# cvxgrp/scs

Measured on AMD Instinct MI355X. Metric: ADMM iters/sec (+ time-to-eps=1e-4), 1e6-var random SOCP, 1 GPU, higher is better.
Workload: dtype f64

## Files before the change

### scs_amd/csrc/linsys.h

```cpp
#pragma once
#include "spmv.h"
#include "scs_host.h"
#include "spmv_wave.h"
#include "spmm.h"

namespace scsamd {

int selected_device();

struct CgCtl {
  real ztr[2];
  real norm_r;
  real tol;
  real rhs_norm;
  int zero_rhs;
  int cg_done;
  int iters;
  int max_its;
  unsigned seq;
};

typedef unsigned long long cg_word;
__host__ __device__ inline cg_word cg_word_pack(unsigned seq, int iters, int done) {
  return ((cg_word)seq << 32) | ((cg_word)(unsigned)iters << 1) | (cg_word)(done ? 1 : 0);
}

struct CgCtlM {
  real ztr[2][MULTI_W_MAX];
  real norm_r[MULTI_W_MAX], tol[MULTI_W_MAX], rhs_norm[MULTI_W_MAX];
  int zero_rhs[MULTI_W_MAX];
  int done[MULTI_W_MAX];
  int iters[MULTI_W_MAX];
  int max_its;
  int all_done;
};

struct MultiWork {
  int width = 0;
  int last_its = 16;
  DevBuf<real> bx, by;
  DevBuf<real> s, r, z, p;
  DevBuf<real> gt;
  DevBuf<real> Pp;
  DevBuf<real> part_pgp, part_ztr, part_max;
  DevBuf<CgCtlM> ctl;
  PinnedBuf<CgCtlM> hctl;
};

struct ShardHook {
  void *ctx = nullptr;
// ... 106 lines not shown
```

### scs_amd/csrc/linsys.hip

```cpp
#include "linsys.h"
#include <thread>
#include <exception>
#include <system_error>
#include <algorithm>
#include "spmv_wave_build.h"
#include "host_transpose.h"
#include <algorithm>
#include <atomic>
#include <chrono>

namespace scsamd {

constexpr int CG_GRAPH_ITERS = 8;
constexpr long long CG_GRAPH_MAX_NNZ = 2000000;
constexpr int CG_LEAD_DEFAULT = 4;
constexpr int CG_PACE_SPIN = 64;


constexpr int VEC_MAX_GRID = 512;
constexpr int PART_CAP = 4096;
static_assert(PART_CAP >= SPMV_MAX_GRID && PART_CAP >= WR_MAX_GRID && PART_CAP >= 2 * 512, "partial arrays too small");

CsrDev::~CsrDev() { delete wave; }

// ... 23 lines not shown

__global__ __launch_bounds__(SCSAMD_BLOCK) void k_rhs_prep(real *b, const real *__restrict__ ry,
                                                           real *tmp, int n, int m,
                                                           const real *part, int pcount, CgCtl *ctl,
                                                           real tol, const real *warm_part,
                                                           int warm_cnt, real warm_scale, int max_its, unsigned seq,
                                                           cg_word *prog) {
  __shared__ real red[4];
  const real nb = reduce_partials_max(part, pcount, red);
  const int gtid = blockIdx.x * blockDim.x + threadIdx.x, gs = gridDim.x * blockDim.x;
  const bool zero = nb <= (real)1e-12;
  if (zero) {
    for (int i = gtid; i < n + m; i += gs) b[i] = 0;
  } else {
    for (int i = gtid; i < m; i += gs) tmp[i] = b[n + i] / ry[i];
  }
  real t = tol;
  if (warm_part) {
    const real nw = reduce_partials_max(warm_part, warm_cnt, red) * warm_scale;
    t = t < nw ? t : nw;
    t = (real)0.2 * t;
    t = t > (real)1e-12 ? t : (real)1e-12;
  }
  if (gtid == 0) {
    ctl->zero_rhs = zero ? 1 : 0;
    ctl->cg_done = zero ? 1 : 0;
    ctl->iters = 0;
    ctl->max_its = max_its;
    ctl->tol = t;
    ctl->rhs_norm = nb;
    ctl->norm_r = 0;
    ctl->ztr[0] = 0;
    ctl->ztr[1] = 0;
    ctl->seq = seq;
    publish_progress(prog, seq, 0, zero ? 1 : 0);
  }
}

__global__ __launch_bounds__(SCSAMD_BLOCK) void k_cg_init(real *x, const real *__restrict__ s, real *r,
                                                          real *z, const real *__restrict__ M, int n,
                                                          real *part_ztr, real *part_max,
                                                          const CgCtl *ctl) {
  __shared__ real red[4];
  if (ctl->zero_rhs) return;
  real ztr = 0, mx = 0;
  for (int i = blockIdx.x * blockDim.x + threadIdx.x; i < n; i += gridDim.x * blockDim.x) {
    real ri;
    if (s) {
      ri = x[i] - r[i];
      x[i] = s[i];
    } else {
      ri = x[i];
      x[i] = 0;
    }
    r[i] = ri;
    const real zi = ri * M[i];
    z[i] = zi;
    ztr += zi * ri;
    const real a = absval(ri);
    mx = a > mx ? a : mx;
  }
  ztr = block_sum(ztr, red);
  mx = block_max(mx, red);
  if (threadIdx.x == 0) {
    part_ztr[blockIdx.x] = ztr;
    part_max[blockIdx.x] = mx;
  }
}

__global__ __launch_bounds__(SCSAMD_BLOCK) void k_cg_start(real *p, const real *__restrict__ z, int n,
                                                           const real *part_ztr, const real *part_max,
                                                           int pcount, CgCtl *ctl, cg_word *prog) {
  __shared__ real red[4];
  if (ctl->zero_rhs) return;
  const real ztr = reduce_partials_sum(part_ztr, pcount, red);
  const real nr = reduce_partials_max(part_max, pcount, red);
  const real tol = ctl->tol;
  const real thr = tol > (real)1e-12 ? tol : (real)1e-12;
  const bool conv = nr < thr;
  if (!conv)
    for (int i = blockIdx.x * blockDim.x + threadIdx.x; i < n; i += gridDim.x * blockDim.x) p[i] = z[i];
  if (blockIdx.x == 0 && threadIdx.x == 0) {
    ctl->ztr[0] = ztr;
    ctl->norm_r = nr;
    if (conv) {
      ctl->cg_done = 1;
      publish_progress(prog, ctl->seq, 0, 1);
    }
  }
}

__global__ __launch_bounds__(SCSAMD_BLOCK) void k_cg_update(real *x, real *r, real *z,
                                                            const real *__restrict__ p,
                                                            const real *__restrict__ Gp,
                                                            const real *__restrict__ M, int n,
                                                            const real *part_pgp, int cnt_pgp,
                                                            real *part_ztr, real *part_max,
                                                            const CgCtl *ctl, int parity, int ntm) {
  __shared__ real red[4];
  const int gtid = blockIdx.x * blockDim.x + threadIdx.x, gs = gridDim.x * blockDim.x;
  const int nv = n / RVW;
  const bool has = gtid < nv;
  rvec P0 = {}, G0 = {}, M0 = {}, X0 = {}, R0 = {};
  if (has) {
    P0 = ldv(p, gtid);
    G0 = ldv(Gp, gtid);
    M0 = ldv(M, gtid);
    X0 = ldv(x, gtid);
    R0 = ldv(r, gtid);
  }
  const int done = ctl->cg_done;
  const real ztr_in = ctl->ztr[parity];
  real psum = 0;
  for (int i = threadIdx.x; i < cnt_pgp; i += blockDim.x) psum += part_pgp[i];
  if (done) return;
  const real pgp = block_sum(psum, red);
  const real alpha = ztr_in / pgp;
  real ztr = 0, mx = 0;
  if (has) {
    rvec Z;
#pragma unroll
    for (int e = 0; e < RVW; ++e) {
      X0.v[e] += alpha * P0.v[e];
      const real ri = R0.v[e] + (-alpha) * G0.v[e];
      R0.v[e] = ri;
      const real zi = ri * M0.v[e];
      Z.v[e] = zi;
      ztr += zi * ri;
      const real a = absval(ri);
      mx = a > mx ? a : mx;
    }
    stv(x, gtid, X0);
    stv(r, gtid, R0);
    stv(z, gtid, Z);
  }
  int iv0 = gtid + gs;
  if (ntm & 4) {
    for (; iv0 + gs < nv; iv0 += 2 * gs) {
      const int ia = iv0, ib = iv0 + gs;
      const rvec Pa = ldv_nt(p, ia), Pb = ldv_nt(p, ib), Ga = ldv_nt(Gp, ia), Gb = ldv_nt(Gp, ib), Ma = ldv_nt(M, ia), Mb = ldv_nt(M, ib);
      rvec Xa = ldv_nt(x, ia), Xb = ldv_nt(x, ib), Ra = ldv_nt(r, ia), Rb = ldv_nt(r, ib), Za, Zb;
#pragma unroll
      for (int e = 0; e < RVW; ++e) {
        Xa.v[e] += alpha * Pa.v[e];
        const real ri = Ra.v[e] + (-alpha) * Ga.v[e];
        Ra.v[e] = ri;
        const real zi = ri * Ma.v[e];
        Za.v[e] = zi;
        ztr += zi * ri;
        const real a = absval(ri);
        mx = a > mx ? a : mx;
      }
#pragma unroll
      for (int e = 0; e < RVW; ++e) {
        Xb.v[e] += alpha * Pb.v[e];
        const real ri = Rb.v[e] + (-alpha) * Gb.v[e];
        Rb.v[e] = ri;
        const real zi = ri * Mb.v[e];
        Zb.v[e] = zi;
        ztr += zi * ri;
        const real a = absval(ri);
        mx = a > mx ? a : mx;
      }
      stv_nt(x, ia, Xa);
      stv_nt(r, ia, Ra);
      stv(z, ia, Za);
      stv_nt(x, ib, Xb);
      stv_nt(r, ib, Rb);
      stv(z, ib, Zb);
    }
  }
  for (int iv = iv0; iv < nv; iv += gs) {
    const rvec P = (ntm & 2) ? ldv_nt(p, iv) : ldv(p, iv), G = (ntm & 2) ? ldv_nt(Gp, iv) : ldv(Gp, iv), Mv = ntm ? ldv_nt(M, iv) : ldv(M, iv);
    rvec X = ntm ? ldv_nt(x, iv) : ldv(x, iv), R = ntm ? ldv_nt(r, iv) : ldv(r, iv), Z;
#pragma unroll
    for (int e = 0; e < RVW; ++e) {
      X.v[e] += alpha * P.v[e];
      const real ri = R.v[e] + (-alpha) * G.v[e];
      R.v[e] = ri;
      const real zi = ri * Mv.v[e];
      Z.v[e] = zi;
      ztr += zi * ri;
      const real a = absval(ri);
      mx = a > mx ? a : mx;
    }
    if (ntm) {
      stv_nt(x, iv, X);
      stv_nt(r, iv, R);
    } else {
      stv(x, iv, X);
      stv(r, iv, R);
    }
    if (ntm & 2) stv_nt(z, iv, Z);
    else stv(z, iv, Z);
  }
  for (int i = nv * RVW + gtid; i < n; i += gs) {
    const real pi = p[i], gi = Gp[i];
    x[i] += alpha * pi;
    const real ri = r[i] + (-alpha) * gi;
    r[i] = ri;
    const real zi = ri * M[i];
    z[i] = zi;
    ztr += zi * ri;
    const real a = absval(ri);
    mx = a > mx ? a : mx;
  }
  ztr = block_sum(ztr, red);
  mx = block_max(mx, red);
  if (threadIdx.x == 0) {
    part_ztr[blockIdx.x] = ztr;
    part_max[blockIdx.x] = mx;
  }
}

__global__ __launch_bounds__(SCSAMD_BLOCK) void k_cg_direction(real *p, const real *__restrict__ z, int n,
                                                               const real *part_ztr,
                                                               const real *part_max, int pcount,
                                                               CgCtl *ctl, int parity, int dmode, cg_word *prog) {
  __shared__ real red[4];
  const int gtid = blockIdx.x * blockDim.x + threadIdx.x, gs = gridDim.x * blockDim.x;
  const int nv = n / RVW;
  const bool has = gtid < nv;
  rvec Z0 = {}, P0 = {};
  if (has) {
    Z0 = ldv(z, gtid);
    P0 = ldv(p, gtid);
  }
  const int done = ctl->cg_done;
  const real ztr_prev = ctl->ztr[parity], tol = ctl->tol;
  real zs = 0, ms = 0;
  for (int i = threadIdx.x; i < pcount; i += blockDim.x) {
    zs += part_ztr[i];
    const real v = part_max[i];
    ms = v > ms ? v : ms;
  }
  if (done) return;
  const real ztr = block_sum(zs, red);
  const real nr = block_max(ms, red);
  const bool conv = nr < tol;
  const bool brk = !conv && ztr_prev == (real)0;
  if (!conv && !brk) {
    const real beta = ztr / ztr_prev;
    if (has) {
#pragma unroll
      for (int e = 0; e < RVW; ++e) P0.v[e] = Z0.v[e] + beta * P0.v[e];
      stv(p, gtid, P0);
    }
    int iv0 = gtid + gs;
    if (dmode & 4) {
      for (; iv0 + gs < nv; iv0 += 2 * gs) {
        const rvec Za = (dmode & 1) ? ldv_nt(z, iv0) : ldv(z, iv0), Zb = (dmode & 1) ? ldv_nt(z, iv0 + gs) : ldv(z, iv0 + gs);
        rvec Pa = ldv(p, iv0), Pb = ldv(p, iv0 + gs);
#pragma unroll
        for (int e = 0; e < RVW; ++e) {
          Pa.v[e] = Za.v[e] + beta * Pa.v[e];
          Pb.v[e] = Zb.v[e] + beta * Pb.v[e];
        }
        stv(p, iv0, Pa);
        stv(p, iv0 + gs, Pb);
      }
    }
    for (int iv = iv0; iv < nv; iv += gs) {
      const rvec Z = (dmode & 1) ? ldv_nt(z, iv) : ldv(z, iv);
      rvec P = ldv(p, iv);
#pragma unroll
      for (int e = 0; e < RVW; ++e) P.v[e] = Z.v[e] + beta * P.v[e];
      if (dmode & 2) stv_nt(p, iv, P);
      else stv(p, iv, P);
    }
    for (int i = nv * RVW + gtid; i < n; i += gs) p[i] = z[i] + beta * p[i];
  }
  if (blockIdx.x == 0 && threadIdx.x == 0) {
    ctl->ztr[parity ^ 1] = ztr;
    ctl->norm_r = nr;
    const int its = ctl->iters + (brk ? 0 : 1);
    const bool stop = conv || brk || its >= ctl->max_its;
    ctl->iters = its;
    if (stop) ctl->cg_done = 1;
    publish_progress(prog, ctl->seq, its, stop ? 1 : 0);
  }
}

__global__ __launch_bounds__(SCSAMD_BLOCK) void k_cg3_update(real *x, real *r, real *p, const real *__restrict__ Gp,
                                                             const real *__restrict__ M, int n, const real *part_pgp,
                                                             const real *part_d1, const real *part_d2, int cnt_sp,
                                                             const real *part_ztr_prev, const real *part_max_prev, int cnt_v,
                                                             real *part_ztr, real *part_max, CgCtl *ctl, int it, cg_word *prog) {
  __shared__ real red[4];
  const int gtid = blockIdx.x * blockDim.x + threadIdx.x, gs = gridDim.x * blockDim.x;
  const int nv = n / RVW;
  const bool has = gtid < nv;
  rvec P0 = {}, G0 = {}, M0 = {}, X0 = {}, R0 = {};
  if (has) {
    P0 = ldv(p, gtid);
    G0 = ldv(Gp, gtid);
    M0 = ldv_nt(M, gtid);
    X0 = ldv_nt(x, gtid);
    R0 = ldv_nt(r, gtid);
  }
  const int done = ctl->cg_done, max_its = ctl->max_its;
  const real tol = ctl->tol;
  real ztr = ctl->ztr[0];
  real s0 = 0, s1 = 0, s2 = 0, zs = 0, ms = 0;
// ... 402 lines not shown
      iters = (int)(it + 1);
    }
  }
  __syncthreads();
  for (int i = tid; i < m; i += FUSED_THREADS) b[n + i] = (-b[n + i] + fused_row(A, b, i)) / ry[i];
  if (tid == 0) {
    ctl->zero_rhs = 0; ctl->cg_done = 1; ctl->iters = iters; ctl->tol = t; ctl->rhs_norm = nb; ctl->norm_r = nr;
    ctl->ztr[0] = ztr; ctl->ztr[1] = 0;
    ctl->seq = seq;
  }
  __syncthreads();
  if (tid == 0) publish_progress(prog, seq, iters, 1);
}

LinSys::~LinSys() {
  if (cg_graph) (void)hipGraphExecDestroy(cg_graph);
  delete multi;
  if (own_stream && stream) (void)hipStreamDestroy(stream);
}

template <int E, int WPB, int MODE>
static void launch_lockstep_one(const WaveRowsDev &wd, int g, size_t lds, hipStream_t stream, const WaveView &v, const real *x, real *y,
                                const EpiArgs &e, const int *skip) {
  static std::atomic<unsigned long long> attr_set[4] = {};
  int dev = 0;
  HIP_CHECK(hipGetDevice(&dev));
  const bool tracked = dev >= 0 && dev < 256;
  const unsigned long long bit = 1ull << (dev & 63);
  if (!tracked || !(attr_set[(dev >> 6) & 3].load(std::memory_order_acquire) & bit)) {
    HIP_CHECK(hipFuncSetAttribute(reinterpret_cast<const void *>(csr_wave_lockstep_kernel<E, WPB, MODE>), hipFuncAttributeMaxDynamicSharedMemorySize,
                                  144 * 1024));
    if (tracked) attr_set[(dev >> 6) & 3].fetch_or(bit, std::memory_order_release);
  }
  hipLaunchKernelGGL((csr_wave_lockstep_kernel<E, WPB, MODE>), dim3(g), dim3(WPB * 64), lds, stream, v, x, y, e, skip, wd.accrows);
}
template <int E>
static void launch_lockstep(const WaveRowsDev &wd, int g, size_t lds, hipStream_t stream, const WaveView &v, const real *x, real *y,
                            const EpiArgs &e, const int *skip) {
#define LS_CASE(W, M)                                                                                                  \
  if (wd.ls_wpb == W && wd.ls_bmode == M) return launch_lockstep_one<E, W, M>(wd, g, lds, stream, v, x, y, e, skip);
  LS_CASE(16, 4) LS_CASE(16, 1) LS_CASE(8, 4) LS_CASE(8, 1)
#undef LS_CASE
  throw HipError("scs_amd: lockstep SpMV variant not instantiated");
}

void LinSys::launch_spmv(int epi, const CsrDev &mat, const real *x, real *y, const EpiArgs &e,
                         const int *skip) {
  int slot = -1;
  const bool sample = profiling && ((spmv_sample_ctr++ % 7) == 0);
  if (sample) slot = spmv_timer.start(stream);
  if (mat.wave && mat.wave->built) {
    const WaveRowsDev &wd = *mat.wave;
    const int g = wd.grid();
    const size_t lds = wd.lds_bytes();
    WaveView v = wd.view();
#define WR_LAUNCH(E)                                                                                                   \
  do {                                                                                                                 \
    if (wd.wide) {                                                                                                     \
      hipLaunchKernelGGL((csr_wave_wide_kernel<E>), dim3(g), dim3(WR_BLOCK), lds, stream, v, x, y, e, skip, wd.accrows);  \
    } else if (wd.lockstep) {                                                                                          \
      launch_lockstep<E>(wd, g, lds, stream, v, x, y, e, skip);                                                        \
    } else if (wd.pipelined == 1) hipLaunchKernelGGL((csr_wave_kernel<E, 1>), dim3(g), dim3(WR_BLOCK), lds, stream, v, x, y, e, skip, wd.accrows); \
    else if (wd.pipelined == 2) hipLaunchKernelGGL((csr_wave_kernel<E, 2>), dim3(g), dim3(WR_BLOCK), lds, stream, v, x, y, e, skip, wd.accrows); \
    else hipLaunchKernelGGL((csr_wave_kernel<E, 0>), dim3(g), dim3(WR_BLOCK), lds, stream, v, x, y, e, skip, wd.accrows);                       \
  } while (0)
    switch (epi) {
    case EPI_PLAIN: WR_LAUNCH(EPI_PLAIN); break;
    case EPI_DIV: WR_LAUNCH(EPI_DIV); break;
    case EPI_GP: WR_LAUNCH(EPI_GP); break;
    case EPI_ACC: WR_LAUNCH(EPI_ACC); break;
    case EPI_NEGDIV: WR_LAUNCH(EPI_NEGDIV); break;
    case EPI_GP3: WR_LAUNCH(EPI_GP3); break;
    default: throw HipError("scs_amd: bad spmv epilogue");
    }
#undef WR_LAUNCH
    if (sample) spmv_timer.stop(slot, stream);
    n_spmv++;
    return;
  }
  const int g = mat.grid();
  CsrView v = mat.view();
  switch (epi) {
  case EPI_PLAIN: hipLaunchKernelGGL(csr_stream_kernel<EPI_PLAIN>, dim3(g), dim3(SCSAMD_BLOCK), 0, stream, v, x, y, e, skip); break;
  case EPI_DIV: hipLaunchKernelGGL(csr_stream_kernel<EPI_DIV>, dim3(g), dim3(SCSAMD_BLOCK), 0, stream, v, x, y, e, skip); break;
  case EPI_GP: hipLaunchKernelGGL(csr_stream_kernel<EPI_GP>, dim3(g), dim3(SCSAMD_BLOCK), 0, stream, v, x, y, e, skip); break;
  case EPI_ACC: hipLaunchKernelGGL(csr_stream_kernel<EPI_ACC>, dim3(g), dim3(SCSAMD_BLOCK), 0, stream, v, x, y, e, skip); break;
  case EPI_NEGDIV: hipLaunchKernelGGL(csr_stream_kernel<EPI_NEGDIV>, dim3(g), dim3(SCSAMD_BLOCK), 0, stream, v, x, y, e, skip); break;
  default: throw HipError("scs_amd: bad spmv epilogue");
  }
  if (sample) spmv_timer.stop(slot, stream);
  n_spmv++;
}

static void host_transpose(int rows_out, int cols_out, const eoff *Ap, const int *Ai, const real *Ax, std::vector<eoff> &Cp, std::vector<int> &Ci,
                           std::vector<real> &Cx, bool force_serial = false) {
  host_transpose_t<eoff, real>(rows_out, cols_out, Ap, Ai, Ax, Cp, Ci, Cx, force_serial);
}
// ... 376 lines not shown
  real *p_cur = pbuf[it & 1];
  if (it == 0) {
    EpiArgs e1{ry.p, nullptr, nullptr, nullptr};
    launch_spmv(EPI_DIV, A, p_cur, tmp.p, e1, &c->cg_done);
  } else {
    const int q = (int)((it - 1) & 1);
    hipLaunchKernelGGL(k_cg2_a, dim3(A.grid()), dim3(SCSAMD_BLOCK), (size_t)n * sizeof(real), stream, A.view(), ry.p, tmp.p, cg_x,
                       rbuf[(it - 1) & 1], rbuf[it & 1], Gp.p, M.p, pbuf[(it - 1) & 1], p_cur, n, partA.p, gAt, gv, c, q, prog_dev);
    n_spmv++;
  }
  EpiArgs e2{rx.p, p_cur, nullptr, partA.p};
  launch_spmv(EPI_GP, At, tmp.p, Gp.p, e2, &c->cg_done);
}

void LinSys::enqueue_cg_iteration(int q) {
  CgCtl *c = ctl.p;
  const int gv = vec_grid(n);
  const int gAt = (At.wave && At.wave->built) ? At.wave->grid() : At.grid();
  real *part_pgp = partA.p, *part_ztr = partB.p, *part_max = partB.p + PART_CAP / 2;
  EpiArgs e1{ry.p, nullptr, nullptr, nullptr};
  launch_spmv(EPI_DIV, A, p.p, tmp.p, e1, &c->cg_done);
  if (has_P) {
    EpiArgs ep{nullptr, nullptr, nullptr, nullptr};
    launch_spmv(EPI_PLAIN, P, p.p, Pp.p, ep, &c->cg_done);
  }
  EpiArgs e2{rx.p, p.p, has_P ? Pp.p : nullptr, shard ? (real *)nullptr : part_pgp};
  launch_spmv(EPI_GP, At, tmp.p, Gp.p, e2, &c->cg_done);
  int cnt_pgp = gAt;
  if (shard) {
    shard_allreduce(Gp.p, (size_t)n, 0);
    hipLaunchKernelGGL(k_dot_partial, dim3(gv), dim3(SCSAMD_BLOCK), 0, stream, (const real *)p.p, (const real *)Gp.p, n, part_pgp, &c->cg_done);
    cnt_pgp = gv;
  }
  hipLaunchKernelGGL(k_cg_update, dim3(gv), dim3(SCSAMD_BLOCK), 0, stream, cg_x, r.p, z.p, p.p, Gp.p, M.p, n,
                     part_pgp, cnt_pgp, part_ztr, part_max, c, q, nt_mode);
  hipLaunchKernelGGL(k_cg_direction, dim3(gv), dim3(SCSAMD_BLOCK), 0, stream, p.p, z.p, n, part_ztr, part_max,
                     gv, c, q, dir_mode, prog_dev);
}

void LinSys::enqueue_cg3_iteration(long long it) {
  CgCtl *c = ctl.p;
  const int gv = vec_grid(n);
  const int gAt = At.wave->grid();
  const int q = (int)(it & 1);
  real *ztr_cur = partB.p + q * (PART_CAP / 4), *max_cur = partB.p + PART_CAP / 2 + q * (PART_CAP / 4);
  real *ztr_prev = partB.p + (q ^ 1) * (PART_CAP / 4), *max_prev = partB.p + PART_CAP / 2 + (q ^ 1) * (PART_CAP / 4);
  EpiArgs e1{ry.p, nullptr, nullptr, nullptr};
  launch_spmv(EPI_DIV, A, p.p, tmp.p, e1, &c->cg_done);
  if (has_P) {
    EpiArgs ep{nullptr, nullptr, nullptr, nullptr};
    launch_spmv(EPI_PLAIN, P, p.p, Pp.p, ep, &c->cg_done);
  }
  EpiArgs e2{rx.p, p.p, has_P ? Pp.p : nullptr, partA.p};
  e2.mv = M.p;
  e2.rv = r.p;
  e2.partial2 = partC.p;
  e2.partial3 = partD.p;
  launch_spmv(EPI_GP3, At, tmp.p, Gp.p, e2, &c->cg_done);
  hipLaunchKernelGGL(k_cg3_update, dim3(gv), dim3(SCSAMD_BLOCK), 0, stream, cg_x, r.p, p.p, Gp.p, M.p, n, partA.p, partC.p, partD.p, gAt,
                     ztr_prev, max_prev, gv, ztr_cur, max_cur, c, (int)std::min<long long>(it, 2147483647LL), prog_dev);
}

bool LinSys::build_cg_graph() {
  cg_graph_tried = true;
  hipGraph_t g = nullptr;
  if (hipStreamBeginCapture(stream, hipStreamCaptureModeRelaxed) != hipSuccess) {
    (void)hipGetLastError();
    return false;
  }
  bool ok = true;
// ... 530 lines not shown
```

### scs_amd/csrc/spmv_wave.h

```cpp
#pragma once
#include "spmv.h"
#include <algorithm>

namespace scsamd {

constexpr int WR_WPB = 4;
constexpr int WR_BLOCK = WR_WPB * 64;
constexpr int WR_ROWS_MAX = 1024;
constexpr int WR_MAX_GRID = 4096;
constexpr int WR_BUCKETS = 1024;

struct WaveView {
  int rows, nunit, cbits, cols;
  const int *urow;
  const eoff *useg;
  const unsigned *wrd;
  const real *val;
  const unsigned short *rowl;
};

#ifdef __HIPCC__
__device__ __forceinline__ void lds_add(real *p, real v) {
  __hip_atomic_fetch_add(p, v, __ATOMIC_RELAXED, __HIP_MEMORY_SCOPE_WORKGROUP);
}

struct WrChunk {
  uint4 w;
  real v[4];
};
__device__ __forceinline__ WrChunk wr_load(const WaveView &A, eoff eb) {
  WrChunk c;
  c.w = *reinterpret_cast<const uint4 *>(A.wrd + eb);
  if (sizeof(real) == 8) {
    const double2 va = *reinterpret_cast<const double2 *>(A.val + eb), vb = *reinterpret_cast<const double2 *>(A.val + eb + 2);
    c.v[0] = (real)va.x; c.v[1] = (real)va.y; c.v[2] = (real)vb.x; c.v[3] = (real)vb.y;
  } else {
    const float4 va = *reinterpret_cast<const float4 *>(A.val + eb);
    c.v[0] = (real)va.x; c.v[1] = (real)va.y; c.v[2] = (real)va.z; c.v[3] = (real)va.w;
  }
  return c;
}
__device__ __forceinline__ void wr_consume(const WaveView &A, const WrChunk &c, const real *__restrict__ x, real *acc, eoff eb, eoff t,
                                           unsigned cmask) {
  const unsigned w[4] = {c.w.x, c.w.y, c.w.z, c.w.w};
  real xx[4];
#pragma unroll
  for (int i = 0; i < 4; ++i) xx[i] = eb + i < t ? x[w[i] & cmask] : (real)0;
#pragma unroll
  for (int i = 0; i < 4; ++i)
    if (eb + i < t) lds_add(acc + (w[i] >> A.cbits), c.v[i] * xx[i]);
}

template <int EPI, int WPB>
__device__ __forceinline__ void wr_block_partials(const EpiArgs &e, real (*red)[WPB], real dot, real d1, real d2, int wave, int lane) {
  dot = wave_sum(dot);
  if (EPI == EPI_GP3) {
    d1 = wave_sum(d1);
    d2 = wave_sum(d2);
  }
  if (lane == 0) {
    red[0][wave] = dot;
    if (EPI == EPI_GP3) {
      red[1][wave] = d1;
      red[2][wave] = d2;
    }
  }
  __syncthreads();
  if (threadIdx.x == 0) {
    real sum = red[0][0];
    for (int i = 1; i < WPB; ++i) sum += red[0][i];
    e.partial[blockIdx.x] = sum;
    if (EPI == EPI_GP3) {
      real s1 = red[1][0], s2 = red[2][0];
      for (int i = 1; i < WPB; ++i) {
        s1 += red[1][i];
        s2 += red[2][i];
      }
      e.partial2[blockIdx.x] = s1;
      e.partial3[blockIdx.x] = s2;
    }
  }
}

template <int EPI, int PIPE>
__global__ __launch_bounds__(WR_BLOCK) void csr_wave_kernel(WaveView A, const real *__restrict__ x, real *y, EpiArgs e,
                                                            const int *skip, int accrows) {
  if (skip && *skip) return;
  extern __shared__ __attribute__((aligned(16))) unsigned char wr_smem[];
  __shared__ real red[3][WR_WPB];
  const int wave = threadIdx.x >> 6, lane = threadIdx.x & 63;
  real *acc = reinterpret_cast<real *>(wr_smem) + (size_t)wave * accrows;
  const unsigned cmask = (1u << A.cbits) - 1;
  real dot = 0, d1 = 0, d2 = 0;
  for (int u = blockIdx.x * WR_WPB + wave; u < A.nunit; u += gridDim.x * WR_WPB) {
    const int r0 = A.urow[u], nr = A.urow[u + 1] - r0;
    const eoff s = A.useg[2 * u], t = A.useg[2 * u + 1];
    for (int k = lane; k < nr; k += 64) acc[k] = 0;
    if (PIPE == 1) {
      WrChunk cur = wr_load(A, s + lane * 4);
      for (eoff e0 = s; e0 < t; e0 += 256) {
        const bool more = e0 + 256 < t;
        WrChunk nxt = cur;
        if (more) nxt = wr_load(A, e0 + 256 + lane * 4);
        wr_consume(A, cur, x, acc, e0 + lane * 4, t, cmask);
        cur = nxt;
      }
    } else if (PIPE == 2) {
      for (eoff e0 = s; e0 < t; e0 += 512) {
        const eoff ea = e0 + lane * 4, eb = ea + 256;
        const bool two = e0 + 256 < t;
        const WrChunk c0 = wr_load(A, ea);
        WrChunk c1 = c0;
        if (two) c1 = wr_load(A, eb);
        const unsigned w0[4] = {c0.w.x, c0.w.y, c0.w.z, c0.w.w}, w1[4] = {c1.w.x, c1.w.y, c1.w.z, c1.w.w};
        real x0[4], x1[4];
#pragma unroll
        for (int i = 0; i < 4; ++i) x0[i] = ea + i < t ? x[w0[i] & cmask] : (real)0;
#pragma unroll
        for (int i = 0; i < 4; ++i) x1[i] = (two && eb + i < t) ? x[w1[i] & cmask] : (real)0;
#pragma unroll
        for (int i = 0; i < 4; ++i)
          if (ea + i < t) lds_add(acc + (w0[i] >> A.cbits), c0.v[i] * x0[i]);
#pragma unroll
        for (int i = 0; i < 4; ++i)
          if (two && eb + i < t) lds_add(acc + (w1[i] >> A.cbits), c1.v[i] * x1[i]);
      }
    } else {
      for (eoff e0 = s; e0 < t; e0 += 256) {
        const eoff eb = e0 + lane * 4;
        const WrChunk c = wr_load(A, eb);
        wr_consume(A, c, x, acc, eb, t, cmask);
      }
    }
    for (int k = lane; k < nr; k += 64) {
      const real a = epi_init<EPI>(e, y, r0 + k) + acc[k];
      if (EPI == EPI_GP3) epi_apply3(e, y, r0 + k, a, dot, d1, d2);
      else epi_apply<EPI>(e, y, r0 + k, a, dot);
    }
  }
  if ((EPI == EPI_GP || EPI == EPI_GP3) && e.partial) wr_block_partials<EPI, WR_WPB>(e, red, dot, d1, d2, wave, lane);
}
template <int EPI>
__global__ __launch_bounds__(WR_BLOCK) void csr_wave_wide_kernel(WaveView A, const real *__restrict__ x, real *y, EpiArgs e, const int *skip,
                                                                 int accrows) {
  if (skip && *skip) return;
  extern __shared__ __attribute__((aligned(16))) unsigned char wr_smem[];
  __shared__ real red[3][WR_WPB];
  const int wave = threadIdx.x >> 6, lane = threadIdx.x & 63;
  real *acc = reinterpret_cast<real *>(wr_smem) + (size_t)wave * accrows;
  real dot = 0, d1 = 0, d2 = 0;
  for (int u = blockIdx.x * WR_WPB + wave; u < A.nunit; u += gridDim.x * WR_WPB) {
    const int r0 = A.urow[u], nr = A.urow[u + 1] - r0;
    const eoff s = A.useg[2 * u], t = A.useg[2 * u + 1];
    for (int k = lane; k < nr; k += 64) acc[k] = 0;
    for (eoff e0 = s; e0 < t; e0 += 256) {
      const eoff eb = e0 + lane * 4;
      const WrChunk c = wr_load(A, eb);
      const uint2 rr = *reinterpret_cast<const uint2 *>(A.rowl + eb);
      const unsigned w[4] = {c.w.x, c.w.y, c.w.z, c.w.w};
      const unsigned lr[4] = {rr.x & 0xffffu, rr.x >> 16, rr.y & 0xffffu, rr.y >> 16};
      real xx[4];
#pragma unroll
      for (int i = 0; i < 4; ++i) xx[i] = eb + i < t ? x[w[i]] : (real)0;
#pragma unroll
      for (int i = 0; i < 4; ++i)
        if (eb + i < t) lds_add(acc + lr[i], c.v[i] * xx[i]);
    }
    for (int k = lane; k < nr; k += 64) {
      const real a = epi_init<EPI>(e, y, r0 + k) + acc[k];
      if (EPI == EPI_GP3) epi_apply3(e, y, r0 + k, a, dot, d1, d2);
      else epi_apply<EPI>(e, y, r0 + k, a, dot);
    }
  }
  if ((EPI == EPI_GP || EPI == EPI_GP3) && e.partial) wr_block_partials<EPI, WR_WPB>(e, red, dot, d1, d2, wave, lane);
}
template <int EPI, int WL_WPB, int MODE, int SLOTS>
__device__ __forceinline__ void wave_lockstep_rounds(const WaveView &A, const real *__restrict__ x, real *y, const EpiArgs &e, real *acc,
                                                     int *s_nch, real &dot, real &d1, real &d2) {
  constexpr bool PRE = SLOTS > 0 && (EPI == EPI_DIV || EPI == EPI_GP);
  constexpr int NS = PRE ? SLOTS : 1;
  const int wave = threadIdx.x >> 6, lane = threadIdx.x & 63;
  const unsigned cmask = (1u << A.cbits) - 1;
  const int per_round = gridDim.x * WL_WPB;
  const int nround = (A.nunit + per_round - 1) / per_round;
  for (int rd = 0; rd < nround; ++rd) {
    const int u = rd * per_round + blockIdx.x * WL_WPB + wave;
    const bool live = u < A.nunit;
    int r0 = 0, nr = 0;
    eoff s = 0, t = 0;
    if (live) {
      r0 = A.urow[u];
      nr = A.urow[u + 1] - r0;
      s = A.useg[2 * u];
      t = A.useg[2 * u + 1];
    }
    for (int k = lane; k < nr; k += 64) acc[k] = 0;
    const int nch = (int)((t - s + 255) >> 8);
    if (lane == 0) s_nch[wave] = nch;
    __syncthreads();
    int nmax = 0;
#pragma unroll
    for (int w = 0; w < WL_WPB; ++w) nmax = s_nch[w] > nmax ? s_nch[w] : nmax;
    constexpr int bars = MODE;
    auto consume = [&](const WrChunk &ch, int c) {
      const eoff eb = s + c * 256 + lane * 4;
      const bool has = c < nch;
      const unsigned w[4] = {ch.w.x, ch.w.y, ch.w.z, ch.w.w};
      real xx[4];
#pragma unroll
      for (int i = 0; i < 4; ++i) {
        if (bars == 4 || (bars == 2 && (i & 1) == 0) || (bars == 1 && i == 0))
          __syncthreads();
        xx[i] = (has && eb + i < t) ? x[w[i] & cmask] : (real)0;
      }
#pragma unroll
      for (int i = 0; i < 4; ++i)
        if (has && eb + i < t) lds_add(acc + (w[i] >> A.cbits), ch.v[i] * xx[i]);
    };
    WrChunk zero;
    zero.w = make_uint4(0, 0, 0, 0);
    zero.v[0] = zero.v[1] = zero.v[2] = zero.v[3] = 0;
    if (PRE) {
      WrChunk ch0 = zero;
      real pd[NS], px[NS], py[NS];
      if (live) {
        ch0 = wr_load(A, s + lane * 4);
        const int rb = __builtin_amdgcn_readfirstlane(r0);
        const real *dp = e.d + rb, *xp = EPI == EPI_GP ? e.xin + rb : nullptr, *yp = EPI == EPI_GP && e.y0 ? e.y0 + rb : nullptr;
// ... 12 lines not shown
      }
#pragma unroll
      for (int j = 0; j < NS; ++j) {
        if (EPI != EPI_GP) px[j] = 0;
        if (!(EPI == EPI_GP && e.y0)) py[j] = 0;
      }
      if (0 < nmax) consume(ch0, 0);
      for (int c = 1; c < nmax; ++c) {
        const WrChunk ch = c < nch ? wr_load(A, s + c * 256 + lane * 4) : zero;
        consume(ch, c);
      }
#pragma unroll
      for (int j = 0; j < NS; ++j) {
        const int k = lane + 64 * j;
        if (k < nr) epi_apply_pre<EPI>(y, r0 + k, py[j] + acc[k], pd[j], px[j], dot);
      }
      for (int k = lane + 64 * NS; k < nr; k += 64) epi_apply<EPI>(e, y, r0 + k, epi_init<EPI>(e, y, r0 + k) + acc[k], dot);
    } else {
      for (int c = 0; c < nmax; ++c) {
        const WrChunk ch = c < nch ? wr_load(A, s + c * 256 + lane * 4) : zero;
        consume(ch, c);
      }
      for (int k = lane; k < nr; k += 64) {
        const real a = epi_init<EPI>(e, y, r0 + k) + acc[k];
        if (EPI == EPI_GP3) epi_apply3(e, y, r0 + k, a, dot, d1, d2);
        else epi_apply<EPI>(e, y, r0 + k, a, dot);
      }
    }
    __syncthreads();
  }
}
template <int EPI, int WL_WPB, int MODE>
__global__ __launch_bounds__(WL_WPB * 64) void csr_wave_lockstep_kernel(WaveView A, const real *__restrict__ x, real *y, EpiArgs e,
                                                                        const int *skip, int accrows) {
  if (skip && *skip) return;
  extern __shared__ __attribute__((aligned(16))) unsigned char wr_smem[];
  __shared__ real red[3][WL_WPB];
  __shared__ int s_nch[WL_WPB];
  const int wave = threadIdx.x >> 6, lane = threadIdx.x & 63;
  real *acc = reinterpret_cast<real *>(wr_smem) + (size_t)wave * accrows;
  real dot = 0, d1 = 0, d2 = 0;
  if (EPI == EPI_DIV || EPI == EPI_GP) {
    const int need = (accrows + 63) >> 6;
    if (need <= 4) wave_lockstep_rounds<EPI, WL_WPB, MODE, 4>(A, x, y, e, acc, s_nch, dot, d1, d2);
    else if (need <= 9 || EPI == EPI_GP) wave_lockstep_rounds<EPI, WL_WPB, MODE, 9>(A, x, y, e, acc, s_nch, dot, d1, d2);
    else wave_lockstep_rounds<EPI, WL_WPB, MODE, 16>(A, x, y, e, acc, s_nch, dot, d1, d2);
  } else {
    wave_lockstep_rounds<EPI, WL_WPB, MODE, 0>(A, x, y, e, acc, s_nch, dot, d1, d2);
  }
  if ((EPI == EPI_GP || EPI == EPI_GP3) && e.partial) wr_block_partials<EPI, WL_WPB>(e, red, dot, d1, d2, wave, lane);
}
#endif

struct WaveRowsDev {
  bool built = false;
  bool built_on_device = false;
  int pipelined = 0;
  double lines_per_entry = 1;
  int rows = 0, cols = 0, nunit = 0, cbits = 0, accrows = 0, cus = 256;
  int lockstep = 0;
  int sub_window_order = 0;
  int ls_wpb = 16, ls_bmode = 4;
  int wpc = 8;
  DevBuf<int> urow;
  DevBuf<eoff> useg;
  long long bias = 0;
  DevBuf<unsigned> wrd;
  DevBuf<real> val;
  bool wide = false;
  DevBuf<unsigned short> rowl;
  WaveView view() const { return WaveView{rows, nunit, cbits, cols, urow.p, useg.p, wrd.p - bias, val.p - bias, wide ? rowl.p - bias : nullptr}; }
  static bool lines_counted(int cols) { return ((long long)cols >> (sizeof(real) == 8 ? 4 : 5)) / 8 <= 64 * 1024; }
  int grid() const {
    const int resident = wpc * cus;
    const int rounds = std::max(1, (nunit + resident - 1) / resident);
    const int per_round = (nunit + rounds - 1) / rounds;
    const int wpb = lockstep ? ls_wpb : WR_WPB;
    return std::max(1, std::min((per_round + wpb - 1) / wpb, WR_MAX_GRID));
  }
  size_t lds_bytes() const { return (size_t)(lockstep ? ls_wpb : WR_WPB) * accrows * sizeof(real); }
  static int col_bits(int cols) {
// ... 211 lines not shown
```

Baseline: 66.74.

## Move CG x-update into direction kernel and prefetch SpMV unit metadata before skip check

The x += alpha*p update moves from the CG update kernel into the direction kernel. The direction kernel already reads p, so the separate load of p in the update pass goes away. Alpha and a liveness flag are now passed through the control struct. Both vector kernels preload CG_AHEAD strided chunks before the control-dependent reductions, which overlaps memory latency with the partial-sum reduction. The wave SpMV kernels now receive per_round and nround from the host and load the first unit's metadata before testing the skip flag, hiding that latency at kernel start. The cost is more register pressure and a few extra control fields.

```diff
diff --git a/scs_amd/csrc/linsys.h b/scs_amd/csrc/linsys.h
--- a/scs_amd/csrc/linsys.h
+++ b/scs_amd/csrc/linsys.h
@@ -13,9 +13,11 @@
   real norm_r;
   real tol;
   real rhs_norm;
+  real alpha;
   int zero_rhs;
   int cg_done;
   int iters;
+  int iter_live;
   int max_its;
   unsigned seq;
 };
diff --git a/scs_amd/csrc/linsys.hip b/scs_amd/csrc/linsys.hip
--- a/scs_amd/csrc/linsys.hip
+++ b/scs_amd/csrc/linsys.hip
@@ -79,6 +79,8 @@
     ctl->norm_r = 0;
     ctl->ztr[0] = 0;
     ctl->ztr[1] = 0;
+    ctl->alpha = 0;
+    ctl->iter_live = 0;
     ctl->seq = seq;
     publish_progress(prog, seq, 0, zero ? 1 : 0);
   }
@@ -137,113 +139,82 @@
   }
 }
 
-__global__ __launch_bounds__(SCSAMD_BLOCK) void k_cg_update(real *x, real *r, real *z,
-                                                            const real *__restrict__ p,
+constexpr int CG_AHEAD = 4;
+__device__ __forceinline__ rvec ldv_pol(const real *p, int iv, bool nt) { return nt ? ldv_nt(p, iv) : ldv(p, iv); }
+__device__ __forceinline__ void stv_pol(real *p, int iv, const rvec &v, bool nt) {
+  if (nt) stv_nt(p, iv, v);
+  else stv(p, iv, v);
+}
+
+__global__ __launch_bounds__(SCSAMD_BLOCK) void k_cg_update(real *r, real *z,
                                                             const real *__restrict__ Gp,
                                                             const real *__restrict__ M, int n,
                                                             const real *part_pgp, int cnt_pgp,
                                                             real *part_ztr, real *part_max,
-                                                            const CgCtl *ctl, int parity, int ntm) {
+                                                            CgCtl *ctl, int parity, int ntm) {
   __shared__ real red[4];
   const int gtid = blockIdx.x * blockDim.x + threadIdx.x, gs = gridDim.x * blockDim.x;
   const int nv = n / RVW;
-  const bool has = gtid < nv;
-  rvec P0 = {}, G0 = {}, M0 = {}, X0 = {}, R0 = {};
-  if (has) {
-    P0 = ldv(p, gtid);
-    G0 = ldv(Gp, gtid);
-    M0 = ldv(M, gtid);
-    X0 = ldv(x, gtid);
-    R0 = ldv(r, gtid);
+  const bool nt_gz = (ntm & 2) != 0, nt_mr = ntm != 0;
+  rvec G[CG_AHEAD], Mv[CG_AHEAD], R[CG_AHEAD];
+#pragma unroll
+  for (int j = 0; j < CG_AHEAD; ++j) {
+    const int iv = gtid + j * gs;
+    G[j] = Mv[j] = R[j] = rvec{};
+    if (iv < nv) {
+      G[j] = ldv_pol(Gp, iv, j > 0 && nt_gz);
+      Mv[j] = ldv_pol(M, iv, j > 0 && nt_mr);
+      R[j] = ldv_pol(r, iv, j > 0 && nt_mr);
+    }
   }
   const int done = ctl->cg_done;
   const real ztr_in = ctl->ztr[parity];
   real psum = 0;
   for (int i = threadIdx.x; i < cnt_pgp; i += blockDim.x) psum += part_pgp[i];
+  if (gtid == 0) ctl->iter_live = done ? 0 : 1;
   if (done) return;
   const real pgp = block_sum(psum, red);
   const real alpha = ztr_in / pgp;
+  if (gtid == 0) ctl->alpha = alpha;
   real ztr = 0, mx = 0;
-  if (has) {
-    rvec Z;
+#pragma unroll
+  for (int j = 0; j < CG_AHEAD; ++j) {
+    const int iv = gtid + j * gs;
+    if (iv < nv) {
+      rvec Z;
+#pragma unroll
+      for (int e = 0; e < RVW; ++e) {
+        const real ri = R[j].v[e] + (-alpha) * G[j].v[e];
+        R[j].v[e] = ri;
+        const real zi = ri * Mv[j].v[e];
+        Z.v[e] = zi;
+        ztr += zi * ri;
+        const real a = absval(ri);
+        mx = a > mx ? a : mx;
+      }
+      stv_pol(r, iv, R[j], j > 0 && nt_mr);
+      stv_pol(z, iv, Z, j > 0 && nt_gz);
+    }
+  }
+  for (long long ivl = (long long)gtid + (long long)CG_AHEAD * gs; ivl < nv; ivl += gs) {
+    const int iv = (int)ivl;
+    const rvec Gv = ldv_pol(Gp, iv, nt_gz), Mc = ldv_pol(M, iv, nt_mr);
+    rvec Rv = ldv_pol(r, iv, nt_mr), Z;
 #pragma unroll
     for (int e = 0; e < RVW; ++e) {
-      X0.v[e] += alpha * P0.v[e];
-      const real ri = R0.v[e] + (-alpha) * G0.v[e];
-      R0.v[e] = ri;
-      const real zi = ri * M0.v[e];
+      const real ri = Rv.v[e] + (-alpha) * Gv.v[e];
+      Rv.v[e] = ri;
+      const real zi = ri * Mc.v[e];
       Z.v[e] = zi;
       ztr += zi * ri;
       const real a = absval(ri);
       mx = a > mx ? a : mx;
     }
-    stv(x, gtid, X0);
-    stv(r, gtid, R0);
-    stv(z, gtid, Z);
-  }
-  int iv0 = gtid + gs;
-  if (ntm & 4) {
-    for (; iv0 + gs < nv; iv0 += 2 * gs) {
-      const int ia = iv0, ib = iv0 + gs;
-      const rvec Pa = ldv_nt(p, ia), Pb = ldv_nt(p, ib), Ga = ldv_nt(Gp, ia), Gb = ldv_nt(Gp, ib), Ma = ldv_nt(M, ia), Mb = ldv_nt(M, ib);
-      rvec Xa = ldv_nt(x, ia), Xb = ldv_nt(x, ib), Ra = ldv_nt(r, ia), Rb = ldv_nt(r, ib), Za, Zb;
-#pragma unroll
-      for (int e = 0; e < RVW; ++e) {
-        Xa.v[e] += alpha * Pa.v[e];
-        const real ri = Ra.v[e] + (-alpha) * Ga.v[e];
-        Ra.v[e] = ri;
-        const real zi = ri * Ma.v[e];
-        Za.v[e] = zi;
-        ztr += zi * ri;
-        const real a = absval(ri);
-        mx = a > mx ? a : mx;
-      }
-#pragma unroll
-      for (int e = 0; e < RVW; ++e) {
-        Xb.v[e] += alpha * Pb.v[e];
-        const real ri = Rb.v[e] + (-alpha) * Gb.v[e];
-        Rb.v[e] = ri;
-        const real zi = ri * Mb.v[e];
-        Zb.v[e] = zi;
-        ztr += zi * ri;
-        const real a = absval(ri);
-        mx = a > mx ? a : mx;
-      }
-      stv_nt(x, ia, Xa);
-      stv_nt(r, ia, Ra);
-      stv(z, ia, Za);
-      stv_nt(x, ib, Xb);
-      stv_nt(r, ib, Rb);
-      stv(z, ib, Zb);
-    }
-  }
-  for (int iv = iv0; iv < nv; iv += gs) {
-    const rvec P = (ntm & 2) ? ldv_nt(p, iv) : ldv(p, iv), G = (ntm & 2) ? ldv_nt(Gp, iv) : ldv(Gp, iv), Mv = ntm ? ldv_nt(M, iv) : ldv(M, iv);
-    rvec X = ntm ? ldv_nt(x, iv) : ldv(x, iv), R = ntm ? ldv_nt(r, iv) : ldv(r, iv), Z;
-#pragma unroll
-    for (int e = 0; e < RVW; ++e) {
-      X.v[e] += alpha * P.v[e];
-      const real ri = R.v[e] + (-alpha) * G.v[e];
-      R.v[e] = ri;
-      const real zi = ri * Mv.v[e];
-      Z.v[e] = zi;
-      ztr += zi * ri;
-      const real a = absval(ri);
-      mx = a > mx ? a : mx;
-    }
-    if (ntm) {
-      stv_nt(x, iv, X);
-      stv_nt(r, iv, R);
-    } else {
-      stv(x, iv, X);
-      stv(r, iv, R);
-    }
-    if (ntm & 2) stv_nt(z, iv, Z);
-    else stv(z, iv, Z);
-  }
-  for (int i = nv * RVW + gtid; i < n; i += gs) {
-    const real pi = p[i], gi = Gp[i];
-    x[i] += alpha * pi;
+    stv_pol(r, iv, Rv, nt_mr);
+    stv_pol(z, iv, Z, nt_gz);
+  }
+  for (long long i = (long long)nv * RVW + gtid; i < n; i += gs) {
+    const real gi = Gp[i];
     const real ri = r[i] + (-alpha) * gi;
     r[i] = ri;
     const real zi = ri * M[i];
@@ -260,21 +231,27 @@
   }
 }
 
-__global__ __launch_bounds__(SCSAMD_BLOCK) void k_cg_direction(real *p, const real *__restrict__ z, int n,
+__global__ __launch_bounds__(SCSAMD_BLOCK) void k_cg_direction(real *p, real *x, const real *__restrict__ z, int n,
                                                                const real *part_ztr,
                                                                const real *part_max, int pcount,
-                                                               CgCtl *ctl, int parity, int dmode, cg_word *prog) {
+                                                               CgCtl *ctl, int parity, int dmode, int ntm, cg_word *prog) {
   __shared__ real red[4];
   const int gtid = blockIdx.x * blockDim.x + threadIdx.x, gs = gridDim.x * blockDim.x;
   const int nv = n / RVW;
-  const bool has = gtid < nv;
-  rvec Z0 = {}, P0 = {};
-  if (has) {
-    Z0 = ldv(z, gtid);
-    P0 = ldv(p, gtid);
-  }
-  const int done = ctl->cg_done;
-  const real ztr_prev = ctl->ztr[parity], tol = ctl->tol;
+  const bool nt_z = (dmode & 1) != 0, nt_p = (dmode & 2) != 0, nt_x = ntm != 0;
+  rvec Z[CG_AHEAD], P[CG_AHEAD], X[CG_AHEAD];
+#pragma unroll
+  for (int j = 0; j < CG_AHEAD; ++j) {
+    const int iv = gtid + j * gs;
+    Z[j] = P[j] = X[j] = rvec{};
+    if (iv < nv) {
+      Z[j] = ldv_pol(z, iv, j > 0 && nt_z);
+      P[j] = ldv(p, iv);
+      X[j] = ldv_pol(x, iv, j > 0 && nt_x);
+    }
+  }
+  const int done = !ctl->iter_live;
+  const real ztr_prev = ctl->ztr[parity], tol = ctl->tol, alpha = ctl->alpha;
   real zs = 0, ms = 0;
   for (int i = threadIdx.x; i < pcount; i += blockDim.x) {
     zs += part_ztr[i];
@@ -286,36 +263,39 @@
   const real nr = block_max(ms, red);
   const bool conv = nr < tol;
   const bool brk = !conv && ztr_prev == (real)0;
-  if (!conv && !brk) {
-    const real beta = ztr / ztr_prev;
-    if (has) {
+  const bool newp = !conv && !brk;
+  const real beta = newp ? ztr / ztr_prev : (real)0;
 #pragma unroll
-      for (int e = 0; e < RVW; ++e) P0.v[e] = Z0.v[e] + beta * P0.v[e];
-      stv(p, gtid, P0);
-    }
-    int iv0 = gtid + gs;
-    if (dmode & 4) {
-      for (; iv0 + gs < nv; iv0 += 2 * gs) {
-        const rvec Za = (dmode & 1) ? ldv_nt(z, iv0) : ldv(z, iv0), Zb = (dmode & 1) ? ldv_nt(z, iv0 + gs) : ldv(z, iv0 + gs);
-        rvec Pa = ldv(p, iv0), Pb = ldv(p, iv0 + gs);
+  for (int j = 0; j < CG_AHEAD; ++j) {
+    const int iv = gtid + j * gs;
+    if (iv < nv) {
 #pragma unroll
-        for (int e = 0; e < RVW; ++e) {
-          Pa.v[e] = Za.v[e] + beta * Pa.v[e];
-          Pb.v[e] = Zb.v[e] + beta * Pb.v[e];
-        }
-        stv(p, iv0, Pa);
-        stv(p, iv0 + gs, Pb);
-      }
-    }
-    for (int iv = iv0; iv < nv; iv += gs) {
-      const rvec Z = (dmode & 1) ? ldv_nt(z, iv) : ldv(z, iv);
-      rvec P = ldv(p, iv);
+      for (int e = 0; e < RVW; ++e) X[j].v[e] += alpha * P[j].v[e];
+      stv_pol(x, iv, X[j], j > 0 && nt_x);
+      if (newp) {
 #pragma unroll
-      for (int e = 0; e < RVW; ++e) P.v[e] = Z.v[e] + beta * P.v[e];
-      if (dmode & 2) stv_nt(p, iv, P);
-      else stv(p, iv, P);
-    }
-    for (int i = nv * RVW + gtid; i < n; i += gs) p[i] = z[i] + beta * p[i];
+        for (int e = 0; e < RVW; ++e) P[j].v[e] = Z[j].v[e] + beta * P[j].v[e];
+        stv_pol(p, iv, P[j], j > 0 && nt_p);
+      }
+    }
+  }
+  for (long long ivl = (long long)gtid + (long long)CG_AHEAD * gs; ivl < nv; ivl += gs) {
+    const int iv = (int)ivl;
+    const rvec Zv = ldv_pol(z, iv, nt_z);
+    rvec Pv = ldv(p, iv), Xv = ldv_pol(x, iv, nt_x);
+#pragma unroll
+    for (int e = 0; e < RVW; ++e) Xv.v[e] += alpha * Pv.v[e];
+    stv_pol(x, iv, Xv, nt_x);
+    if (newp) {
+#pragma unroll
+      for (int e = 0; e < RVW; ++e) Pv.v[e] = Zv.v[e] + beta * Pv.v[e];
+      stv_pol(p, iv, Pv, nt_p);
+    }
+  }
+  for (long long i = (long long)nv * RVW + gtid; i < n; i += gs) {
+    const real pi = p[i];
+    x[i] += alpha * pi;
+    if (newp) p[i] = z[i] + beta * pi;
   }
   if (blockIdx.x == 0 && threadIdx.x == 0) {
     ctl->ztr[parity ^ 1] = ztr;
@@ -784,7 +764,9 @@
                                   144 * 1024));
     if (tracked) attr_set[(dev >> 6) & 3].fetch_or(bit, std::memory_order_release);
   }
-  hipLaunchKernelGGL((csr_wave_lockstep_kernel<E, WPB, MODE>), dim3(g), dim3(WPB * 64), lds, stream, v, x, y, e, skip, wd.accrows);
+  const int per_round = g * WPB;
+  hipLaunchKernelGGL((csr_wave_lockstep_kernel<E, WPB, MODE>), dim3(g), dim3(WPB * 64), lds, stream, v, x, y, e, skip, wd.accrows, per_round,
+                     std::max(1, (wd.nunit + per_round - 1) / per_round));
 }
 template <int E>
 static void launch_lockstep(const WaveRowsDev &wd, int g, size_t lds, hipStream_t stream, const WaveView &v, const real *x, real *y,
@@ -812,9 +794,9 @@
       hipLaunchKernelGGL((csr_wave_wide_kernel<E>), dim3(g), dim3(WR_BLOCK), lds, stream, v, x, y, e, skip, wd.accrows);  \
     } else if (wd.lockstep) {                                                                                          \
       launch_lockstep<E>(wd, g, lds, stream, v, x, y, e, skip);                                                        \
-    } else if (wd.pipelined == 1) hipLaunchKernelGGL((csr_wave_kernel<E, 1>), dim3(g), dim3(WR_BLOCK), lds, stream, v, x, y, e, skip, wd.accrows); \
-    else if (wd.pipelined == 2) hipLaunchKernelGGL((csr_wave_kernel<E, 2>), dim3(g), dim3(WR_BLOCK), lds, stream, v, x, y, e, skip, wd.accrows); \
-    else hipLaunchKernelGGL((csr_wave_kernel<E, 0>), dim3(g), dim3(WR_BLOCK), lds, stream, v, x, y, e, skip, wd.accrows);                       \
+    } else if (wd.pipelined == 1) hipLaunchKernelGGL((csr_wave_kernel<E, 1>), dim3(g), dim3(WR_BLOCK), lds, stream, v, x, y, e, skip, wd.accrows, g * WR_WPB); \
+    else if (wd.pipelined == 2) hipLaunchKernelGGL((csr_wave_kernel<E, 2>), dim3(g), dim3(WR_BLOCK), lds, stream, v, x, y, e, skip, wd.accrows, g * WR_WPB); \
+    else hipLaunchKernelGGL((csr_wave_kernel<E, 0>), dim3(g), dim3(WR_BLOCK), lds, stream, v, x, y, e, skip, wd.accrows, g * WR_WPB);                       \
   } while (0)
     switch (epi) {
     case EPI_PLAIN: WR_LAUNCH(EPI_PLAIN); break;
@@ -1257,10 +1239,10 @@
     hipLaunchKernelGGL(k_dot_partial, dim3(gv), dim3(SCSAMD_BLOCK), 0, stream, (const real *)p.p, (const real *)Gp.p, n, part_pgp, &c->cg_done);
     cnt_pgp = gv;
   }
-  hipLaunchKernelGGL(k_cg_update, dim3(gv), dim3(SCSAMD_BLOCK), 0, stream, cg_x, r.p, z.p, p.p, Gp.p, M.p, n,
+  hipLaunchKernelGGL(k_cg_update, dim3(gv), dim3(SCSAMD_BLOCK), 0, stream, r.p, z.p, Gp.p, M.p, n,
                      part_pgp, cnt_pgp, part_ztr, part_max, c, q, nt_mode);
-  hipLaunchKernelGGL(k_cg_direction, dim3(gv), dim3(SCSAMD_BLOCK), 0, stream, p.p, z.p, n, part_ztr, part_max,
-                     gv, c, q, dir_mode, prog_dev);
+  hipLaunchKernelGGL(k_cg_direction, dim3(gv), dim3(SCSAMD_BLOCK), 0, stream, p.p, cg_x, z.p, n, part_ztr, part_max,
+                     gv, c, q, dir_mode, nt_mode, prog_dev);
 }
 
 void LinSys::enqueue_cg3_iteration(long long it) {
diff --git a/scs_amd/csrc/spmv_wave.h b/scs_amd/csrc/spmv_wave.h
--- a/scs_amd/csrc/spmv_wave.h
+++ b/scs_amd/csrc/spmv_wave.h
@@ -23,6 +23,23 @@
 __device__ __forceinline__ void lds_add(real *p, real v) {
   __hip_atomic_fetch_add(p, v, __ATOMIC_RELAXED, __HIP_MEMORY_SCOPE_WORKGROUP);
 }
+
+struct WrUnit {
+  int r0, r1;
+  eoff s, t;
+};
+__device__ __forceinline__ WrUnit wr_unit(const WaveView &A, int u) {
+  WrUnit d;
+  d.r0 = A.urow[u];
+  d.r1 = A.urow[u + 1];
+  d.s = A.useg[2 * u];
+  d.t = A.useg[2 * u + 1];
+  return d;
+}
+__device__ __forceinline__ int wr_skip_word(const int *skip) {
+  return skip ? __hip_atomic_load(skip, __ATOMIC_RELAXED, __HIP_MEMORY_SCOPE_AGENT) : 0;
+}
+template <typename T> __device__ __forceinline__ void wr_arg_now(T v) { asm volatile("" ::"s"(v)); }
 
 struct WrChunk {
   uint4 w;
@@ -84,17 +101,25 @@
 
 template <int EPI, int PIPE>
 __global__ __launch_bounds__(WR_BLOCK) void csr_wave_kernel(WaveView A, const real *__restrict__ x, real *y, EpiArgs e,
-                                                            const int *skip, int accrows) {
-  if (skip && *skip) return;
+                                                            const int *skip, int accrows, int per_round) {
+  const int wave = threadIdx.x >> 6, lane = threadIdx.x & 63;
+  int u = blockIdx.x * WR_WPB + wave;
+  wr_arg_now(x);
+  wr_arg_now(y);
+  wr_arg_now(accrows);
+  wr_arg_now(per_round);
+  const int skw = wr_skip_word(skip);
+  WrUnit un = {0, 0, 0, 0};
+  if (u < A.nunit) un = wr_unit(A, u);
+  if (__builtin_amdgcn_readfirstlane(skw)) return;
   extern __shared__ __attribute__((aligned(16))) unsigned char wr_smem[];
   __shared__ real red[3][WR_WPB];
-  const int wave = threadIdx.x >> 6, lane = threadIdx.x & 63;
   real *acc = reinterpret_cast<real *>(wr_smem) + (size_t)wave * accrows;
   const unsigned cmask = (1u << A.cbits) - 1;
   real dot = 0, d1 = 0, d2 = 0;
-  for (int u = blockIdx.x * WR_WPB + wave; u < A.nunit; u += gridDim.x * WR_WPB) {
-    const int r0 = A.urow[u], nr = A.urow[u + 1] - r0;
-    const eoff s = A.useg[2 * u], t = A.useg[2 * u + 1];
+  while (u < A.nunit) {
+    const int r0 = un.r0, nr = un.r1 - un.r0;
+    const eoff s = un.s, t = un.t;
     for (int k = lane; k < nr; k += 64) acc[k] = 0;
     if (PIPE == 1) {
       WrChunk cur = wr_load(A, s + lane * 4);
@@ -137,6 +162,8 @@
       if (EPI == EPI_GP3) epi_apply3(e, y, r0 + k, a, dot, d1, d2);
       else epi_apply<EPI>(e, y, r0 + k, a, dot);
     }
+    u += per_round;
+    if (u < A.nunit) un = wr_unit(A, u);
   }
   if ((EPI == EPI_GP || EPI == EPI_GP3) && e.partial) wr_block_partials<EPI, WR_WPB>(e, red, dot, d1, d2, wave, lane);
 }
@@ -176,24 +203,22 @@
 }
 template <int EPI, int WL_WPB, int MODE, int SLOTS>
 __device__ __forceinline__ void wave_lockstep_rounds(const WaveView &A, const real *__restrict__ x, real *y, const EpiArgs &e, real *acc,
-                                                     int *s_nch, real &dot, real &d1, real &d2) {
+                                                     int *s_nch, real &dot, real &d1, real &d2, const WrUnit &first, int per_round,
+                                                     int nround) {
   constexpr bool PRE = SLOTS > 0 && (EPI == EPI_DIV || EPI == EPI_GP);
   constexpr int NS = PRE ? SLOTS : 1;
   const int wave = threadIdx.x >> 6, lane = threadIdx.x & 63;
   const unsigned cmask = (1u << A.cbits) - 1;
-  const int per_round = gridDim.x * WL_WPB;
-  const int nround = (A.nunit + per_round - 1) / per_round;
   for (int rd = 0; rd < nround; ++rd) {
     const int u = rd * per_round + blockIdx.x * WL_WPB + wave;
     const bool live = u < A.nunit;
-    int r0 = 0, nr = 0;
-    eoff s = 0, t = 0;
-    if (live) {
-      r0 = A.urow[u];
-      nr = A.urow[u + 1] - r0;
-      s = A.useg[2 * u];
-      t = A.useg[2 * u + 1];
-    }
+    WrUnit un = first;
+    if (rd > 0) {
+      un = WrUnit{0, 0, 0, 0};
+      if (live) un = wr_unit(A, u);
+    }
+    const int r0 = un.r0, nr = un.r1 - un.r0;
+    const eoff s = un.s, t = un.t;
     for (int k = lane; k < nr; k += 64) acc[k] = 0;
     const int nch = (int)((t - s + 255) >> 8);
     if (lane == 0) s_nch[wave] = nch;
@@ -272,21 +297,30 @@
 }
 template <int EPI, int WL_WPB, int MODE>
 __global__ __launch_bounds__(WL_WPB * 64) void csr_wave_lockstep_kernel(WaveView A, const real *__restrict__ x, real *y, EpiArgs e,
-                                                                        const int *skip, int accrows) {
-  if (skip && *skip) return;
+                                                                        const int *skip, int accrows, int per_round, int nround) {
+  const int wave = threadIdx.x >> 6, lane = threadIdx.x & 63;
+  const int u0 = blockIdx.x * WL_WPB + wave;
+  wr_arg_now(x);
+  wr_arg_now(y);
+  wr_arg_now(accrows);
+  wr_arg_now(per_round);
+  wr_arg_now(nround);
+  const int skw = wr_skip_word(skip);
+  WrUnit first = {0, 0, 0, 0};
+  if (u0 < A.nunit) first = wr_unit(A, u0);
+  if (__builtin_amdgcn_readfirstlane(skw)) return;
   extern __shared__ __attribute__((aligned(16))) unsigned char wr_smem[];
   __shared__ real red[3][WL_WPB];
   __shared__ int s_nch[WL_WPB];
-  const int wave = threadIdx.x >> 6, lane = threadIdx.x & 63;
   real *acc = reinterpret_cast<real *>(wr_smem) + (size_t)wave * accrows;
   real dot = 0, d1 = 0, d2 = 0;
   if (EPI == EPI_DIV || EPI == EPI_GP) {
     const int need = (accrows + 63) >> 6;
-    if (need <= 4) wave_lockstep_rounds<EPI, WL_WPB, MODE, 4>(A, x, y, e, acc, s_nch, dot, d1, d2);
-    else if (need <= 9 || EPI == EPI_GP) wave_lockstep_rounds<EPI, WL_WPB, MODE, 9>(A, x, y, e, acc, s_nch, dot, d1, d2);
-    else wave_lockstep_rounds<EPI, WL_WPB, MODE, 16>(A, x, y, e, acc, s_nch, dot, d1, d2);
+    if (need <= 4) wave_lockstep_rounds<EPI, WL_WPB, MODE, 4>(A, x, y, e, acc, s_nch, dot, d1, d2, first, per_round, nround);
+    else if (need <= 9 || EPI == EPI_GP) wave_lockstep_rounds<EPI, WL_WPB, MODE, 9>(A, x, y, e, acc, s_nch, dot, d1, d2, first, per_round, nround);
+    else wave_lockstep_rounds<EPI, WL_WPB, MODE, 16>(A, x, y, e, acc, s_nch, dot, d1, d2, first, per_round, nround);
   } else {
-    wave_lockstep_rounds<EPI, WL_WPB, MODE, 0>(A, x, y, e, acc, s_nch, dot, d1, d2);
+    wave_lockstep_rounds<EPI, WL_WPB, MODE, 0>(A, x, y, e, acc, s_nch, dot, d1, d2, first, per_round, nround);
   }
   if ((EPI == EPI_GP || EPI == EPI_GP3) && e.partial) wr_block_partials<EPI, WL_WPB>(e, red, dot, d1, d2, wave, lane);
 }
```

Measured after the change: 67.68 (median of 5 runs). Within noise of the previous version (+1.4%).
